# akosiorek/sqair

Measured on AMD Instinct MI355X. Metric: frames/sec (forward IWAE ELBO, 10-step 50x50 moving glyphs, K=5), higher is better.
Workload: dtype f32; 1 GPU; cfg2: T=10 HxW=50x50 B=32/GPU K=5 N=4 cells VanillaRNN/GRU/GRU forward (elbo_iwae), HIP-graph replay=True; global_batch=32, seq_len=10, parallelism=dp1, graph_nodes=879

## Files before the change

### sqair_amd/_capi.py

```python
from __future__ import annotations

import ctypes as C
import os

_HERE = os.path.dirname(os.path.abspath(__file__))
LIB_PATH = os.path.join(_HERE, "libsqair_hip.so")

OUTPUT_FIELDS = [
    "what", "what_loc", "what_scale", "where", "where_loc", "where_scale", "presence_prob", "presence",
    "presence_logit", "obj_id", "step_log_prob", "canvas", "glimpse", "disc_what_log_prob",
    "disc_where_log_prob", "disc_what_prior_log_prob", "disc_where_prior_log_prob", "disc_log_prob",
    "disc_prior_log_prob", "disc_prob", "prop_what_log_prob", "prop_where_log_prob",
    "prop_what_prior_log_prob", "prop_where_prior_log_prob", "prop_log_prob", "prop_prior_log_prob",
    "prop_prob", "discrete_log_prob", "num_prop_steps_per_sample", "num_disc_steps_per_sample",
    "num_steps_per_sample", "prop_pres", "disc_pres", "data_ll_per_sample", "kl_per_sample",
    "log_q_z_given_x_per_sample", "log_p_z_per_sample", "log_weights_per_timestep",
    "final_temporal_state", "final_prior_state", "final_last_used_id",
]
N_REFERENCE_OUTPUTS = 38


class SqairConfig(C.Structure):
    _fields_ = [
        ("img_h", C.c_int32), ("img_w", C.c_int32), ("glimpse_size", C.c_int32),
# ... 126 lines not shown
    "sqair_fill_noise": (C.c_int, [C.c_void_p, C.c_void_p, C.c_int, C.c_int, C.c_int, C.c_int, C.c_uint64, C.c_uint64, C.c_void_p]),
    "sqair_capture_begin": (C.c_int, [C.c_void_p, C.c_void_p]),
    "sqair_capture_end": (C.c_int, [C.c_void_p, C.c_void_p, C.c_int]),
    "sqair_capture_launch": (C.c_int, [C.c_void_p, C.c_int, C.c_void_p]),
    "sqair_add_l2_grad": (C.c_int, [C.c_void_p, C.c_void_p, C.c_void_p, C.c_int64, C.c_float, C.c_void_p]),
    "sqair_rmsprop_step": (C.c_int, [C.c_void_p, C.c_void_p, C.c_void_p, C.c_void_p, C.c_void_p, C.c_int64, C.c_float,
                                     C.c_float, C.c_float, C.c_float, C.c_float, C.c_void_p]),
    "sqair_linear_bwd_test": (C.c_int, [C.c_void_p] * 8 + [C.c_int] * 4 + [C.c_void_p, C.c_int64, C.c_void_p]),
    "sqair_debug_linear_time": (C.c_int, [C.c_void_p, C.c_void_p, C.c_void_p, C.c_void_p, C.c_void_p, C.c_int, C.c_int, C.c_int, C.c_int,
                                          C.c_void_p, C.c_int64, C.c_int, C.POINTER(C.c_float), C.c_void_p]),
    "sqair_debug_linear_graph_time": (C.c_int, [C.c_void_p, C.c_void_p, C.c_void_p, C.c_void_p, C.c_void_p, C.c_int, C.c_int, C.c_int, C.c_int,
                                              C.c_void_p, C.c_int64, C.c_int, C.c_int, C.c_int, C.POINTER(C.c_float), C.c_void_p]),
    "sqair_debug_dense_log": (C.c_int, [C.c_void_p, C.c_int]),
    "sqair_debug_dense_log_entry": (C.c_int, [C.c_void_p, C.c_int, C.POINTER(C.c_int)]),
    "sqair_debug_specialised_launches": (C.c_int64, []),
    "sqair_debug_layers": (C.c_int, [C.c_void_p]),
    "sqair_debug_padded_count": (C.c_int64, [C.c_void_p, C.POINTER(C.c_int)]),
    "sqair_debug_layer": (C.c_int, [C.c_void_p, C.c_int, C.POINTER(C.c_int), C.POINTER(C.c_int),
                                    C.POINTER(C.c_int), C.POINTER(C.c_int), C.POINTER(C.c_int)]),
    "sqair_debug_plan": (C.c_int, [C.c_void_p, C.c_int, C.POINTER(C.c_int), C.POINTER(C.c_int),
                                   C.POINTER(C.c_int)]),
}

EXPORTED_SYMBOLS = [n for n in _PROTOS if not n.startswith("sqair_debug")]

TIMELINE_LIB_PATH = os.path.join(_HERE, "libsqair_hip_timeline.so")
WIDE_LIB_PATH = os.path.join(_HERE, "libsqair_hip_wide.so")
PRODUCT_LIMITS = dict(n_what=50, n_steps_per_image=8, n_hidden=256)
WIDE_LIMITS = dict(n_what=128, n_steps_per_image=14, n_hidden=512)

# ... 74 lines not shown
```

### sqair_amd/csrc/sqair_api.hip

```cpp
#include <algorithm>
#include <mutex>
#include <set>
#include <utility>

#include "sqair_internal.h"
#include "sqair_chain.h"

void sq_set_error(SqairHandle* h, const std::string& msg) {
  if (h) h->err = msg;
}

struct PDim {
  std::vector<std::pair<int, int>> seg;
  PDim(int n) { seg.push_back({n, n}); }
  PDim(int t, int p) { seg.push_back({t, p}); }
  int t() const { int n = 0; for (auto& s : seg) n += s.first; return n; }
  int p() const { int n = 0; for (auto& s : seg) n += s.second; return n; }
  std::vector<int> map() const {
    std::vector<int> m;
    int base = 0;
    for (auto& s : seg) { for (int i = 0; i < s.first; ++i) m.push_back(base + i); base += s.second; }
    return m;
  }
};
// ... 173 lines not shown
  r[rec::PRES] = pres_row;
  return r;
}

struct SegSrc {
  std::string w;
  RowMap rows;
};
struct ColBlock {
  int ncols;
  int col0;
  std::vector<SegSrc> seg;
  std::string bias_a, bias_b;
};

static void build_layer(SqairHandle* h, LayerId id, const std::vector<int>& seg_width, const std::vector<ColBlock>& blocks) {
  PackedLayer& L = h->layers[id];
  L.seg_width = seg_width;
  L.kc = 0;
  for (int w : seg_width) L.kc += (w + 15) / 16;
  L.N = 0;
  for (const ColBlock& b : blocks) L.N += b.ncols;
  L.nt = (L.N + 15) / 16;
  L.w_off = h->packed_w;
  L.b_off = h->packed_b;
  const int64_t nel = (int64_t)L.nt * L.kc * 256;
  h->widx.resize(h->packed_w + nel, -1);
  h->bidx_a.resize(h->packed_b + L.nt * 16, -1);
  h->bidx_b.resize(h->packed_b + L.nt * 16, -1);
  int n0 = 0;
  for (const ColBlock& b : blocks) {
// ... 26 lines not shown
          for (int k = 0; k < seg_width[s]; ++k) {
            if (src.rows[k] < 0) continue;
            const int c = cbase + k / 16, kin = k % 16;
            const int lane = (kin / 4) * 16 + ln, comp = kin % 4;
            h->widx[L.w_off + (((int64_t)tile * L.kc + c) * 64 + lane) * 4 + comp] =
                (int)(woff + (int64_t)src.rows[k] * ldw + b.col0 + j);
          }
        }
        cbase += nch;
      }
    }
    n0 += b.ncols;
  }
  h->packed_w += nel;
  h->packed_b += L.nt * 16;
}

static ColBlock cb1(int ncols, int col0, const std::string& w, const RowMap& rows, const std::string& ba = "",
                    const std::string& bb = "") {
  ColBlock b;
  b.ncols = ncols;
  b.col0 = col0;
  b.seg.push_back({w, rows});
  b.bias_a = ba;
  b.bias_b = bb;
  return b;
}

static void build_plan(SqairHandle* h) {
  const SqairConfig& c = h->cfg;
// ... 49 lines not shown
    build_layer(h, L_PRIOR_GRU2, {nh}, {cb1(16, 0, "prop.prior_rnn.h2h.w", rm_none(nh))});
  } else {
    const RowMap zx = rm_zrec(nw, nw, 0, -1);
    std::vector<ColBlock> bl;
    const char* g[3] = {"z", "r", "h"};
    for (int i = 0; i < 3; ++i) {
      ColBlock b;
      b.ncols = nh;
      b.col0 = 0;
      b.seg.push_back({std::string("prop.prior_gru.w") + g[i], zx});
      if (i < 2) b.seg.push_back({std::string("prop.prior_gru.u") + g[i], rm_range(0, nh)});
      else b.seg.push_back({"", RowMap()});
      b.bias_a = std::string("prop.prior_gru.b") + g[i];
      bl.push_back(b);
    }
    build_layer(h, L_PRIOR_GRU1, {rec::ZW, nh}, bl);
    simple(L_PRIOR_GRU2, "prop.prior_gru.uh", nh, nh, 0, false);
  }
  simple(L_PRIOR_LIN, "prop.prior_linear", nh, 2 * (4 + nw) + 1);
  build_layer(h, L_TAU1, {nh},
              {cb1(128, 0, "prop.where_bias.l0.w", rm_range(0, nh), "prop.where_bias.l0.b"),
               cb1(128, 0, "enc.mask.l0.w", rm_range(0, nh), "enc.mask.l0.b")});
  simple(L_WB2, "prop.where_bias.l1", 128, 4);
  simple(L_MASK2, "enc.mask.l1", 128, G2);
  simple(L_GENC0, "enc.glimpse.l0", G2, nh);
  simple(L_GENC1, "enc.glimpse.l1", nh, nh);
  build_layer(h, L_WHAT_LOC, {nh}, {cb1(nw, 0, "enc.what_head.w", rm_range(0, nh), "enc.what_head.b")});
  simple(L_WHAT_HEAD, "enc.what_head", nh, 2 * nw);
  {
    std::vector<ColBlock> bl;
    for (int cc = 0; cc < nw; ++cc) {
// ... 19 lines not shown
    if (c.time_cell == CELL_VANILLA) {
      ColBlock u;
      u.ncols = nh; u.col0 = 0;
      u.seg = {{"", RowMap()}, {"", RowMap()}, {"prop.temporal_rnn.h2h.w", rm_range(0, nh)}};
      u.bias_a = "prop.temporal_rnn.i2h.b"; u.bias_b = "prop.temporal_rnn.h2h.b";
      bl.push_back(u);
    }
    for (const char* g : {"z", "r"}) {
      if (c.time_cell != CELL_GRU) break;
      ColBlock u;
      u.ncols = nh; u.col0 = 0;
      u.seg = {{"", RowMap()}, {"", RowMap()}, {std::string("prop.temporal_gru.u") + g, rm_range(0, nh)}};
      u.bias_a = std::string("prop.temporal_gru.b") + g;
      bl.push_back(u);
    }
    build_layer(h, L_PRE, {nw, rec::ZW, nh}, bl);
  }
  {
    build_layer(h, L_PROP_RNN, {rec::ZW, nh}, rnn_blocks("prop", {rm_zrec(nw, nw + nw, nw, nw + nw + 4), RowMap()}, 1, false, fin_p));
    if (RG) simple(L_PROP_RNN2, "prop.rnn_gru.uh", nh, nh, 0, false);
    else build_layer(h, L_PROP_RNN2, {nh}, {cb1(16, 0, "prop.what_head.w", rm_none(nh))});
  }
  build_layer(h, L_PROP_T1, {nh},
              {cb1(nh, 0, "prop.transform.l0.w", rm_range(0, nh)), cb1(nsp, 0, "prop.steps.l0.w", rm_range(0, nh))});
  simple(L_PROP_T2, "prop.transform.l1", nh, nh);
  simple(L_PROP_T3, "prop.transform.l2", nh, 8);
  if (c.time_cell == CELL_LSTM) {
    const std::string w = "prop.temporal_lstm.w";
    const int fin = nh + 4 + 2 * nw;
    ColBlock b;
    b.ncols = 4 * nh; b.col0 = 0;
// ... 340 lines not shown
  w.chain_ctl = (unsigned*)take(w.chain ? (int64_t)SQ_CHAIN_MAX_LAUNCHES * SQ_CHAIN_CTL_WORDS : 64);
  w.total = o;
  return w;
}
static Workspace carve(const SqairHandle* h, int T, int B, float* base) { return sq_carve(h, T, B, base, false); }

extern "C" int64_t sqair_workspace_bytes(const SqairHandle* h, int T, int B) {
  if (!h || T < 1 || B < 1) return -1;
  return sq_carve(h, T, B, nullptr, false).total * 4;
}
extern "C" int64_t sqair_train_workspace_bytes(const SqairHandle* h, int T, int B) {
  if (!h || T < 1 || B < 1) return -1;
  return sq_carve(h, T, B, nullptr, true).total * 4;
}

int sq_run(SqairHandle* h, Lin& l, LayerId id, int M, const float* packed, hipStream_t s) {
  const PackedLayer& L = h->layers[id];
  const PackedLayout pl = packed_layout(h);
  if (l.a.nseg != (int)L.seg_width.size()) {
    sq_set_error(h, "internal: segment count mismatch in layer " + std::to_string((int)id));
    return -3;
  }
  for (int i = 0; i < l.a.nseg; ++i)
    if (l.a.seg[i].width != L.seg_width[i]) {
      sq_set_error(h, "internal: segment width mismatch in layer " + std::to_string((int)id));
      return -3;
    }
  l.a.wp = packed + pl.w + L.w_off;
  l.a.wzero = packed + pl.w;
  l.a.bias = packed + pl.b + L.b_off;
  l.a.M = M;
  l.a.N = L.N;
  if (h->dense_log_on) { const int e[4] = {(int)id, M, L.kc * 16, L.N}; h->dense_log.insert(h->dense_log.end(), e, e + 4); }
  if (sq_chain_active(h)) return sq_chain_add_dense(h, l.a, L.kc, L.nt);
  const int rc = sq_launch_linear(l.a, L, s);
  if (rc != 0) sq_set_error(h, "internal: A-operand contract (16-byte aligned, ld % 4 == 0) violated in layer " + std::to_string((int)id));
  return rc;
}

static bool can_fuse_tail(const SqairHandle* h, LayerId id) {
  const PackedLayer& L = h->layers[id];
  const int nh = h->cfg.n_hidden;
  return h->cfg.rnn_cell == RNN_VANILLA && (nh == 128 || nh == 256) && L.seg_width.size() == 2 && L.seg_width[0] == rec::ZW &&
         L.seg_width[1] == nh && L.kc == 4 + nh / 16 && L.nt == nh / 16 && L.N == nh && h->opt_tail_fusion;
}
static int run_rnn_tail(SqairHandle* h, const TailArgs& ta, Dims d, LayerId id, const float* hid, int hid_ld, const float* add, int add_ld,
                        float* out, int out_ld, const float* packed, hipStream_t s) {
  const PackedLayer& L = h->layers[id];
  const PackedLayout pl = packed_layout(h);
  if (h->dense_log_on) { const int e[4] = {-1 - (int)id, d.R, L.kc * 16, L.N}; h->dense_log.insert(h->dense_log.end(), e, e + 4); }
// ... 351 lines not shown
    }
    if (w.chain) {
      const int rc = sq_chain_flush(h, w.chain_ctl + (size_t)(2 * t) * SQ_CHAIN_CTL_WORDS, 2 * t, s);
      if (rc != 0) return rc;
    }
    const bool do_generate = c.sample_from_prior && c.generate_after > 0 && (t_offset + t) > c.generate_after;
    GenArgs ga; memset(&ga, 0, sizeof(ga));
    if (c.sample_from_prior) {
      ga.rec_p = rec_p_t; ga.rec_d = rec_d_t; ga.rec_prev = rec_prev; ga.pstats = pstats_t; ga.ps_ld = PS_LD; ga.spre = spre_t;
      ga.gen_noise = h->gen_noise + (size_t)t * R * 2 * N * nzw; ga.gen = w.gen + (size_t)t * M * gen::W; ga.flat = flat;
      ga.do_generate = do_generate ? 1 : 0; ga.cfg = c;
      sq_launch_generate_prop(ga, po, d, s);
    }
    {
      Lin a; a.seg(rec_p_t, RW, rec::ZW).out(lea, nh).act(ACT_ELU); RUN(a, L_LAT0, M);
      Lin b; b.seg(lea, nh, nh).out(leb, nh).act(ACT_ELU); RUN(b, L_LAT1, M);
      sq_launch_latent_sum(leb, rec_p_t, cvec, d, s);
      Lin p; p.seg(cvec, nh, nh).add(w.pre_disc + (size_t)t * B * rw, rw, rw, K).out(w.pre_d, rw); RUN(p, L_PRED, R);
      if (c.rec_where_prior) {
        Lin q; q.seg(w.rn_init_state, 0, 4).seg(cvec, nh, nh).out(spre_t, 128); RUN(q, L_RNCOND, R);
      }
    }
    if (w.chain) sq_chain_begin(h, d, po, wsbase, ws_bytes);
    for (int j = 0; j < N; ++j) {
      {
        CropArgs ca; memset(&ca, 0, sizeof(ca));
        ca.mode = CROP_DISC;
        const int rc = slot_front(disc, j, ca, !fw);
        if (rc != 0) return rc;
      }
      if (fw) {
        const int rc = run_what(h, 0, w.slot(w.e2, nh, t, 1, j), w.sld(nh), R, j, nz, nullptr, 0, nullptr, rec_d_t, packed, s);
// ... 210 lines not shown
  if (h) sq_set_error(h, "sqair_timeline_begin: this library was built without -DSQAIR_TIMELINE (use libsqair_hip_timeline.so)");
  return -3;
}
extern "C" int sqair_timeline_count(const SqairHandle*) { return -3; }
extern "C" int sqair_timeline_end(SqairHandle*) { return -3; }
extern "C" int sqair_timeline_record(const SqairHandle*, int, const char**, int64_t*, int*, int*) { return -3; }
#endif

extern "C" int sqair_set_option(SqairHandle* h, const char* name, int value) {
  if (!h || !name) return -1;
  const std::string n(name);
  if (n == "tail_fusion") { h->opt_tail_fusion = value != 0; return 0; }
  if (n == "what_fusion") { h->opt_what_fusion = value != 0; return 0; }
  if (n == "specialised") { h->opt_specialised = value != 0; return 0; }
  if (n == "specialised_mask") { h->opt_specialised_mask = value; return 0; }
  if (n == "vi_target") {
    if (value != 0 && value != 1) { sq_set_error(h, "sqair_set_option: vi_target is 0 (vimco) or 1 (reinforce)"); return -2; }
    h->opt_vi_target = value;
    return 0;
  }
  if (n == "slot_chain") {
#ifdef SQAIR_WIDE
    if (value != 0) { sq_set_error(h, "sqair_set_option: slot_chain is not available in the wide build"); return -2; }
#endif
    h->opt_slot_chain = value != 0;
    h->opt_slot_chain_mode = value;
    return 0;
  }
  if (n == "slot_chain_arena_kb") {
    if (sq_chain_set_arena_kb(h, value) != 0) { sq_set_error(h, "sqair_set_option: slot_chain_arena_kb is 64 .. 1048576, set before the first pass"); return -2; }
    return 0;
  }
  sq_set_error(h, "sqair_set_option: unknown option '" + n + "' (known: tail_fusion, what_fusion, specialised, specialised_mask, slot_chain, slot_chain_arena_kb, vi_target)");
  return -2;
}

__global__ __launch_bounds__(256) void k_finite_check(const float* __restrict__ x, int64_t n, int* __restrict__ flag SQ_TLP) {
  SQ_TL_SCOPE;
  int bad = 0;
  int64_t first = n;
  for (int64_t i = (int64_t)blockIdx.x * 256 + threadIdx.x; i < n; i += (int64_t)gridDim.x * 256) {
    const float v = x[i];
    if (!(fabsf(v) <= 3.4028234664e38f)) { ++bad; if (i < first) first = i; }
  }
  if (bad) {
    atomicAdd(&flag[0], bad);
    atomicMin(&flag[1], (int)(first < 0x7fffffff ? first : 0x7fffffff));
  }
// ... 455 lines not shown
  hipStream_t s = (hipStream_t)stream;
  Dims d = make_dims(h->cfg, B);
  d.spec = h->opt_specialised && sq_spec_ok(d) ? (h->opt_specialised_mask & SPEC_ALL) : 0;
  CompactArgs ka; memset(&ka, 0, sizeof(ka));
  ka.rec_p = rec_p; ka.rec_d = rec_d; ka.rec_prev = rec_prev; ka.temporal_p = temporal_p; ka.prior_p = prior_p;
  ka.last_id_prev = last_id_prev; ka.last_id_next = last_id_next;
  ka.rec_next = rec_next; ka.temporal_next = temporal_next; ka.prior_next = prior_next;
  ka.flat = flat; ka.t = t; ka.out = *out; ka.src_out = src_out;
  sq_launch_compact(ka, h->po, d, s);
  SQ_CHECK_HIP(hipGetLastError());
  SQ_CHECK_HIP(hipStreamSynchronize(s));
  return 0;
}

extern "C" int64_t sqair_debug_specialised_launches(void) { return (int64_t)sq_spec_launches(); }
extern "C" int sqair_debug_layers(const SqairHandle* h) { return h ? (int)L_COUNT : -1; }
extern "C" int64_t sqair_debug_padded_count(const SqairHandle* h, int* u2i) {
  if (!h) return -1;
  if (u2i) memcpy(u2i, h->u2i.data(), h->u2i.size() * sizeof(int));
  return h->n_params;
}
extern "C" int sqair_debug_layer(const SqairHandle* h, int id, int* kc, int* nt, int* n, int* nseg, int* seg_widths) {
  if (!h || id < 0 || id >= L_COUNT) return -1;
  const PackedLayer& L = h->layers[id];
  *kc = L.kc; *nt = L.nt; *n = L.N; *nseg = (int)L.seg_width.size();
  for (size_t i = 0; i < L.seg_width.size() && i < 4; ++i) seg_widths[i] = L.seg_width[i];
  return 0;
}
extern "C" int sqair_debug_plan(const SqairHandle* h, int id, int* widx, int* bidx_a, int* bidx_b) {
  if (!h || id < 0 || id >= L_COUNT) return -1;
// ... 156 lines not shown
```

### sqair_amd/csrc/sqair_common.h

```cpp
#pragma once
#include <hip/hip_runtime.h>
#include <stdint.h>
#include <string>
#include <vector>

#include "../../include/sqair_hip.h"

#define SQ_CHECK_HIP(expr)                                                                   \
  do {                                                                                       \
    hipError_t _e = (expr);                                                                  \
    if (_e != hipSuccess) {                                                                  \
      sq_set_error(h, std::string(#expr) + ": " + hipGetErrorString(_e));                    \
      return -2;                                                                             \
    }                                                                                        \
  } while (0)

namespace rec {
#ifdef SQAIR_WIDE
constexpr int NWMAX = 128;
constexpr int WHERE = 0;
constexpr int WHAT = 4;
constexpr int PRES = 132;
constexpr int LOGIT = 133;
constexpr int ZW = 134;
// ... 58 lines not shown
  const float* e0; int e0_ld;
  const float* e1; int e1_ld;
  float* o1; int o1_ld;
  float* o2; int o2_ld;
  float* o3; int o3_ld;
  int nh;
};

struct PackedLayer {
  int64_t w_off;
  int64_t b_off;
  int kc;
  int nt;
  int N;
  std::vector<int> seg_width;
};

struct SqairHandle;
void sq_set_error(SqairHandle* h, const std::string& msg);
int sq_allow_big_lds(const void* kernel, int bytes);

__device__ __forceinline__ void philox4x32_10(unsigned c0, unsigned c1, unsigned c2, unsigned c3, unsigned k0, unsigned k1,
                                              unsigned out[4]) {
#pragma unroll
  for (int r = 0; r < 10; ++r) {
    const unsigned long long p0 = (unsigned long long)0xD2511F53u * c0, p1 = (unsigned long long)0xCD9E8D57u * c2;
    const unsigned n0 = (unsigned)(p1 >> 32) ^ c1 ^ k0, n1 = (unsigned)p1, n2 = (unsigned)(p0 >> 32) ^ c3 ^ k1, n3 = (unsigned)p0;
    c0 = n0; c1 = n1; c2 = n2; c3 = n3;
    k0 += 0x9E3779B9u; k1 += 0xBB67AE85u;
  }
  out[0] = c0; out[1] = c1; out[2] = c2; out[3] = c3;
}

int sq_launch_linear(const LinArgs& a, const PackedLayer& L, hipStream_t s);
int sq_launch_pack(const float* flat, float* packed_w, const int* idx, int64_t n, hipStream_t s);
int sq_launch_pack_bias(const float* flat, float* packed_b, const int* idxa, const int* idxb, int64_t n,
                        hipStream_t s);

#ifdef SQAIR_TIMELINE
struct SqTl { unsigned long long* slot; unsigned gx, gy, nw, pad; };
SqTl sq_tl_next(const char* kernel, dim3 grid, dim3 block);
#define SQ_TLP , const SqTl sq_tl
#define SQ_TL_SCOPE SqTlScope sq_tl_scope(sq_tl)
#define SQ_LAUNCH(kern, grid, block, lds, s, ...) \
  hipLaunchKernelGGL(kern, grid, block, lds, s, __VA_ARGS__, sq_tl_next(#kern, grid, block))
#ifdef __HIPCC__
struct SqTlScope {
  const SqTl tl;
  const unsigned long long t0;
// ... 151 lines not shown
```

### sqair_amd/csrc/sqair_glue.hip

```cpp
#include <atomic>

#include "sqair_glue.h"
#include "sqair_rowops.h"
#include "sqair_canvas.h"

__global__ void k_init_state(float* __restrict__ rec_m, float* __restrict__ temporal_m, float* __restrict__ prior_m,
                             float* __restrict__ last_id, float* __restrict__ disc_init_rec,
                             float* __restrict__ prop_rnn_init, float* __restrict__ disc_rnn_init,
                             float* __restrict__ rn_init_state, float* __restrict__ w3_prop,
                             float* __restrict__ w3_disc, int w3p_off, int w3d_off,
                             const float* __restrict__ flat, POff po, Dims d SQ_TLP) {
  SQ_TL_SCOPE;
  const int rs = blockIdx.x;
  const int tid = threadIdx.x;
  for (int i = tid; i < rec::W; i += blockDim.x) rec_m[(size_t)rs * rec::W + i] = (i == rec::ID) ? -1.0f : 0.0f;
  for (int i = tid; i < d.snh; i += blockDim.x) temporal_m[(size_t)rs * d.snh + i] = flat[po.temporal_init + i];
  for (int i = tid; i < d.psnh; i += blockDim.x) prior_m[(size_t)rs * d.psnh + i] = flat[po.prior_init + i];
  if (tid == 0 && (rs % d.N) == 0) last_id[rs / d.N] = -1.0f;
  if (rs == 0) {
    if (tid == 0) disc_init_rec[rec::PRES] = 1.0f;
    for (int i = tid; i < d.rsnh; i += blockDim.x) {
      prop_rnn_init[i] = flat[po.prop_rnn_init + i];
      disc_rnn_init[i] = flat[po.disc_rnn_init + i];
    }
// ... 835 lines not shown
  const dim3 g(nt, mt);
  if (d.nh == 256) SQ_RT(4, 1);
  else if (d.nh == 128) SQ_RT(2, 1);
  else return -1;
#undef SQ_RT
  return 0;
#endif
}

__global__ void k_latent_sum(const float* __restrict__ f, const float* __restrict__ rec_p, float* __restrict__ c, Dims d SQ_TLP) {
  SQ_TL_SCOPE;
  const int r = blockIdx.x;
  for (int n = threadIdx.x; n < d.nh; n += blockDim.x) {
    float acc = 0.0f;
    for (int k = 0; k < d.N; ++k)
      acc += f[((size_t)r * d.N + k) * d.nh + n] * rec_p[((size_t)r * d.N + k) * rec::W + rec::PRES];
    c[(size_t)r * d.nh + n] = acc;
  }
}
int sq_launch_latent_sum(const float* f, const float* rec_p, float* c, Dims d, hipStream_t s) {
  SQ_LAUNCH(k_latent_sum, dim3(d.R), dim3(256), 0, s, f, rec_p, c, d);
  return 0;
}

constexpr int SQ_LOGPROB_WAVES = 2;
__global__ __launch_bounds__(64 * SQ_LOGPROB_WAVES) void k_logprob(const LogprobArgs a, const POff po, const Dims d SQ_TLP) {
  SQ_TL_SCOPE;
  extern __shared__ __attribute__((aligned(16))) float smem[];
  const int r = blockIdx.x;
  const int fr = blockIdx.y;
  const int tid = threadIdx.x;
// ... 1203 lines not shown
```

### sqair_amd/csrc/sqair_internal.h

```cpp
#pragma once
#include <cstdio>
#include <cstring>
#include <map>

#include "sqair_glue.h"

struct ParamEntry {
  std::string name;
  int64_t off, numel;
  int rows, cols;
};

enum LayerId {
  L_IENC0, L_IENC1, L_PREDISC, L_PRIOR_GRU1, L_PRIOR_GRU2, L_PRIOR_LIN, L_TAU1, L_WB2, L_MASK2, L_GENC0, L_GENC1,
  L_WHAT_LOC, L_WHAT_HEAD, L_PRE, L_PROP_RNN, L_PROP_T1, L_PROP_T2, L_PROP_T3, L_PROP_GRU1, L_PROP_GRU2,
  L_PROP_HEADS, L_PROP_S1, L_LAT0, L_LAT1, L_PRED, L_RNCOND, L_DISC_RNN, L_DISC_T1, L_DISC_T2, L_DISC_T3,
  L_DISC_S1, L_DEC0, L_DEC1, L_DEC2, L_PROP_RNN2, L_DISC_RNN2,
  L_WHAT_HEAD_I, L_PROP_HEADS_I,
  L_COUNT
};

struct SqairHandle {
  SqairConfig cfg;
  SqairConfig ucfg;
// ... 18 lines not shown
  int64_t packed_w = 0, packed_b = 0;
  bool plan_uploaded_to = false;
  const void* plan_uploaded_ptr = nullptr;
  hipGraph_t graph = nullptr;
  hipGraphExec_t graph_exec = nullptr;
  int graph_nodes = 0;
  int debug_reps = 0;
  int debug_graph_nodes = 0;
  bool debug_graph_dependent = false;
  bool dense_log_on = false;
  std::vector<int> dense_log;
  float debug_us = 0.0f;
  bool opt_what_fusion = true;
  bool opt_specialised = true;
  int opt_specialised_mask = 3;
  bool opt_tail_fusion = true;
  bool opt_slot_chain = false;
  int opt_slot_chain_mode = 0;
  int opt_vi_target = 0;
  void* chain = nullptr;
  bool clear_each_pass = true;
  const float* gen_noise = nullptr;
  bool state_on = false;
  const void* state_in = nullptr;
  void* state_out = nullptr;
  const int32_t* state_src = nullptr;
  int state_B = 0;
  bool smc_on = false;
  SqairSmc smc = {};
  bool hist_on = false;
// ... 131 lines not shown
                                 int* t_row, float* fresh, int t0);
SQ_LOCAL int sq_history_refusal(SqairHandle* h, int T, int B, const SqairOutputs* outp);
SQ_LOCAL int sq_observed_refusal(SqairHandle* h, bool train, int T);
SQ_LOCAL HistPushArgs sq_history_push_args(const SqairHandle* h, const SqStateRes& st, const SqairOutputs& out, const int* t_row, int T, int B);
SQ_LOCAL SmcArgs sq_smc_args(const SqairSmc& m, const float* lw, const int32_t* t_row, int T, int B, int K);
SQ_LOCAL int sq_prior_step(SqairHandle* h, const float* packed, hipStream_t s, int M, const float* rec_prev, const float* prior_prev,
                           float* prior_p, float* pgz, float* pgrh, float* pgxh, float* pstats, float* o3, float* o1);

void sq_zero_fill(float* p, int64_t n, hipStream_t s);
void sq_copy(float* dst, const float* src, int64_t n, hipStream_t s);

inline const float* sq_flat(const SqairHandle* h, const float* user_flat, const void* packed) {
  return h->padded ? (const float*)packed + packed_layout(h).fi : user_flat;
}
void sq_flat_gather(const SqairHandle* h, const float* padded_grad, float* user_grad, const void* packed, hipStream_t s);
int sq_run(SqairHandle* h, Lin& l, LayerId id, int M, const float* packed, hipStream_t s);
#define RUN(l, id, M)                                   \
  do {                                                  \
    int _rc = sq_run(h, (l), (id), (M), packed, s);     \
    if (_rc != 0) return _rc;                           \
  } while (0)
```

### sqair_amd/csrc/sqair_linear.hip

```cpp
#include <type_traits>
#include "sqair_common.h"
#include "sqair_lin_device.h"
#include <stdio.h>
#include <stdlib.h>

typedef float f32x4 __attribute__((ext_vector_type(4)));

__global__ void k_pack(const float* __restrict__ flat, float* __restrict__ packed, const int* __restrict__ idx,
                       int64_t n SQ_TLP) {
  SQ_TL_SCOPE;
  constexpr int U = 8;
  int64_t i = (int64_t)blockIdx.x * blockDim.x + threadIdx.x;
  const int64_t stride = (int64_t)gridDim.x * blockDim.x;
  for (; i < n; i += stride * U) {
    int j[U];
    float v[U];
#pragma unroll
    for (int u = 0; u < U; ++u) j[u] = idx[min(i + u * stride, n - 1)];
#pragma unroll
    for (int u = 0; u < U; ++u) v[u] = flat[max(j[u], 0)];
#pragma unroll
    for (int u = 0; u < U; ++u)
      if (i + u * stride < n) packed[i + u * stride] = j[u] >= 0 ? v[u] : 0.0f;
  }
// ... 15 lines not shown
  if (blocks > 4096) blocks = 4096;
  SQ_LAUNCH(k_pack, dim3(blocks), dim3(256), 0, s, flat, packed_w, idx, n);
  return 0;
}
int sq_launch_pack_bias(const float* flat, float* packed_b, const int* idxa, const int* idxb, int64_t n,
                        hipStream_t s) {
  if (n <= 0) return 0;
  SQ_LAUNCH(k_pack_bias, dim3((unsigned)((n + 255) / 256)), dim3(256), 0, s, flat, packed_b, idxa, idxb, n);
  return 0;
}


#define SQ_KLINEAR_NAME k_linear
#include "sqair_linear_kernel.inc"
#undef SQ_KLINEAR_NAME

template <int NCH>
__global__ __launch_bounds__(256) void k_linear_rows(const LinArgs a, const int kc_total, const int n_tiles SQ_TLP) {
  SQ_TL_SCOPE;
  const int tid = threadIdx.x;
  const int wave = tid >> 6;
  const int lane = tid & 63;
  const int tile_n = blockIdx.x;
  const int tile_m = blockIdx.y * 4 + wave;
  (void)n_tiles;
  const int arow = min(tile_m * 16 + (lane & 15), a.M - 1);
  const int kq = lane >> 4;

  const int n = tile_n * 16 + (lane & 15);
  const int nc = min(n, a.N - 1);
// ... 669 lines not shown
  const dim3 g(L.nt, (a.M + 15) / 16);
#define SQ_LAUNCH_KL(G) SQ_LAUNCH((k_linear<NCH, NSEG, G>), g, dim3(256), 0, s, a.seg[0].p, a.wp, a.seg[0].ld, a.seg[0].width, a.seg[0].rmul, a.M, L.kc, L.nt, a.wzero, a)
  if (a.epi == EPI_ACT) SQ_LAUNCH_KL(false); else SQ_LAUNCH_KL(true);
#undef SQ_LAUNCH_KL
}
template <int NCH>
static void launch_nch(const LinArgs& a, const PackedLayer& L, hipStream_t s) {
  switch (a.nseg) {
    case 1: launch_seg<NCH, 1>(a, L, s); break;
    case 2: launch_seg<NCH, 2>(a, L, s); break;
    case 3: launch_seg<NCH, 3>(a, L, s); break;
    default: launch_seg<NCH, 4>(a, L, s); break;
  }
}

static unsigned rmul_of(int rdiv) { return rdiv <= 1 ? 0u : (unsigned)((1ull << 32) / (unsigned)rdiv) + 1u; }

int sq_launch_linear(const LinArgs& a_in, const PackedLayer& L, hipStream_t s) {
  LinArgs a = a_in;
  for (int i = 0; i < a.nseg; ++i) a.seg[i].rmul = rmul_of(a.seg[i].rdiv);
  a.add_rmul = rmul_of(a.add_rdiv);
  const int mt = (a.M + 15) / 16;
  const int grid = mt * L.nt;
  if (grid <= 0) return 0;
  for (int i = 0; i < a.nseg; ++i) {
    const LinSeg& sg = a.seg[i];
    if ((reinterpret_cast<uintptr_t>(sg.p) & 15) != 0 || (sg.ld & 3) != 0 || sg.width < 1 || sg.rdiv < 1) return -5;
  }
#ifndef SQAIR_MT_ROWS_DEFAULT
#define SQAIR_MT_ROWS_DEFAULT 6000
#endif
  static const int mt_rows = SQ_KNOB_INT("SQAIR_MT_ROWS", SQAIR_MT_ROWS_DEFAULT);
  const bool mid_wide = L.kc > 4 && a.M >= 1792 && L.nt >= 48;
// ... 27 lines not shown
    if (((a.M + 127) / 128) * ((L.nt + 3) / 4) >= lds_wgs) {
      SQ_LAUNCH((k_linear_lds<2>), dim3((L.nt + 3) / 4, (a.M + 127) / 128), dim3(256), 0, s, a, L.kc, L.nt);
      return 0;
    }
    const MtShape sh = pick_mt_shape(a.M, L.nt, L.kc);
    if (sh.nt >= 2) launch_mt<4, 1, 2>(a, L, mt, sh.coal != 0, s);
    else launch_mt<4, 1, 1>(a, L, mt, sh.coal != 0, s);
    return 0;
  }
  const int per_wave = (L.kc + 3) / 4;
  static const int t2_rows = SQ_KNOB_INT("SQAIR_T2_ROWS", 512), t2_kc = SQ_KNOB_INT("SQAIR_T2_KC", 40);
  if (a.M >= t2_rows && L.nt >= 4 && L.kc >= t2_kc) {
    launch_t2_any(a, L, s);
    return 0;
  }
  switch (per_wave) {
    case 1: launch_nch<1>(a, L, s); break;
    case 2: launch_nch<2>(a, L, s); break;
    case 3: launch_nch<3>(a, L, s); break;
    case 4: launch_nch<4>(a, L, s); break;
    case 5: launch_nch<5>(a, L, s); break;
    case 6: launch_nch<6>(a, L, s); break;
    case 7: launch_nch<7>(a, L, s); break;
    case 8: launch_nch<8>(a, L, s); break;
    case 9: launch_nch<9>(a, L, s); break;
    default: launch_nch<10>(a, L, s); break;
  }
  return 0;
}
```

### sqair_amd/csrc/sqair_linear_kernel.inc

```
template <int NCH, int NSEG = 4, bool GRU = true>
__global__ __launch_bounds__(256) void SQ_KLINEAR_NAME(const float* __restrict__ p0, const float* __restrict__ wp0, const int ld0,
                                                const int width0, const unsigned rmul0, const int M0, const int kc_total,
                                                const int n_tiles, const float* __restrict__ wzero0, const LinArgs a SQ_TLP) {
  SQ_TL_SCOPE;
  __shared__ float red[4 * 256];
  const int tid = threadIdx.x;
  const int wave = tid >> 6;
  const int lane = tid & 63;
#if defined(SQ_ROWTILE_XCD_AFFINITY)
  const int xcd = blockIdx.x & 7, qq = blockIdx.x >> 3;
  const int tile_n = qq % n_tiles;
  const int tile_m = xcd + 8 * (qq / n_tiles);
  if (tile_m * 16 >= a.M) return;
#else
  const int tile_n = blockIdx.x;
  const int tile_m = blockIdx.y;
  (void)n_tiles;
#endif
  const int arow = min(tile_m * 16 + (lane & 15), M0 - 1);
  const int kq = lane >> 4;

  const f32x4* __restrict__ wp = reinterpret_cast<const f32x4*>(wp0) + ((size_t)tile_n * kc_total) * 64 + lane;
  const int nmine = (kc_total - wave + 3) >> 2;
  const f32x4* __restrict__ wz = reinterpret_cast<const f32x4*>(wzero0) + lane;
  f32x4 av[NCH], bv[NCH];
#ifdef SQ_ABL_NO_B
#define SQ_KL_LOADB(p) f32x4{1.0f, 1.0f, 1.0f, 1.0f}
#else
#define SQ_KL_LOADB(p) *(p)
#endif
#define SQ_KL_ISSUE_B(BASE)                                                                                      \
  _Pragma("unroll") for (int j = 0; j < NCH; ++j) {                                                              \
    const bool valid = (BASE) + j < nmine;                                                                       \
    const int g = valid ? wave + 4 * ((BASE) + j) : wave;                                                        \
    bv[j] = SQ_KL_LOADB(valid ? wp + (size_t)g * 64 : wz);  \
  }
  if (NSEG > 1) {
    SQ_KL_ISSUE_B(0)
    __builtin_amdgcn_sched_barrier(0);
  }

  int cum1 = 0x7fffffff, cum2 = 0x7fffffff, cum3 = 0x7fffffff;
#define SQ_ROWOF(sg) ((sg).rmul ? (int)__umulhi((unsigned)arow, (sg).rmul) : arow)
  const float* rp0 = p0 + (size_t)(rmul0 ? (int)__umulhi((unsigned)arow, rmul0) : arow) * ld0;
  const float* rp1 = rp0; const float* rp2 = rp0; const float* rp3 = rp0;
  int lim0 = ((width0 + 3) & ~3) - 4, lim1 = 0, lim2 = 0, lim3 = 0;
  {
    int c = (width0 + 15) >> 4;
    if (NSEG > 1 && a.nseg > 1) { cum1 = c; c += (a.seg[1].width + 15) >> 4; rp1 = a.seg[1].p + (size_t)SQ_ROWOF(a.seg[1]) * a.seg[1].ld; lim1 = ((a.seg[1].width + 3) & ~3) - 4; }
    if (NSEG > 2 && a.nseg > 2) { cum2 = c; c += (a.seg[2].width + 15) >> 4; rp2 = a.seg[2].p + (size_t)SQ_ROWOF(a.seg[2]) * a.seg[2].ld; lim2 = ((a.seg[2].width + 3) & ~3) - 4; }
    if (NSEG > 3 && a.nseg > 3) { cum3 = c; rp3 = a.seg[3].p + (size_t)SQ_ROWOF(a.seg[3]) * a.seg[3].ld; lim3 = ((a.seg[3].width + 3) & ~3) - 4; }
  }

#undef SQ_ROWOF
  f32x4 acc0 = {0.0f, 0.0f, 0.0f, 0.0f}, acc1 = {0.0f, 0.0f, 0.0f, 0.0f};
#ifdef SQ_ABL_NO_A
#define SQ_KL_LOADA(p) f32x4{1.0f, 1.0f, 1.0f, 1.0f}
#else
#define SQ_KL_LOADA(p) *reinterpret_cast<const f32x4*>(p)
#endif
#define SQ_KL_ISSUE(BASE, FIRST)                                                                                 \
  _Pragma("unroll") for (int j = 0; j < NCH; ++j) {                                                              \
    const bool valid = (BASE) + j < nmine;                                                                       \
    const int g = valid ? wave + 4 * ((BASE) + j) : wave;  \
    const bool s1 = NSEG > 1 && g >= cum1, s2 = NSEG > 2 && g >= cum2, s3 = NSEG > 3 && g >= cum3;  \
    const float* rp = s3 ? rp3 : (s2 ? rp2 : (s1 ? rp1 : rp0));                                                  \
    const int cb = s3 ? cum3 : (s2 ? cum2 : (s1 ? cum1 : 0));                                                    \
    const int lim = s3 ? lim3 : (s2 ? lim2 : (s1 ? lim1 : lim0));                                                \
    av[j] = SQ_KL_LOADA(rp + min((g - cb) * 16 + kq * 4, lim));                                                  \
    if (!((FIRST) && NSEG > 1)) bv[j] = SQ_KL_LOADB(valid ? wp + (size_t)g * 64 : wz);                           \
  }
#ifndef SQ_ABL_NO_MFMA
#define SQ_KL_MFMA()                                                                                             \
  _Pragma("unroll") for (int j = 0; j < NCH; ++j) {                                                              \
    acc0 = __builtin_amdgcn_mfma_f32_16x16x4f32(av[j].x, bv[j].x, acc0, 0, 0, 0);                                \
    acc1 = __builtin_amdgcn_mfma_f32_16x16x4f32(av[j].y, bv[j].y, acc1, 0, 0, 0);                                \
    acc0 = __builtin_amdgcn_mfma_f32_16x16x4f32(av[j].z, bv[j].z, acc0, 0, 0, 0);                                \
    acc1 = __builtin_amdgcn_mfma_f32_16x16x4f32(av[j].w, bv[j].w, acc1, 0, 0, 0);                                \
  }
// ... 12 lines not shown
  const bool g2 = GRU && a.epi == EPI_GRU2;
  const int mcd = a.add_rmul ? (int)__umulhi((unsigned)mc, a.add_rmul) : mc;
  const float* pa = use_add ? a.add + (size_t)mcd * a.add_ld + nc : pb;
  const float* pe0 = g1 ? a.e0 + (size_t)mc * a.e0_ld + (nc - a.nh) : (g2 ? a.e0 + (size_t)mc * a.e0_ld + nc : pb);
  const float* pe1 = g2 ? a.e1 + (size_t)mc * a.e1_ld + nc : pb;
  const float* psc = a.scale_ptr != nullptr ? a.scale_ptr : pb;
#ifdef SQ_ABL_NO_EPI
  const float p_bias = 0.0f; float p_add = 0.0f; const float p_e0 = 0.0f, p_e1 = 0.0f; float p_scale = 1.0f;
  (void)pa; (void)pe0; (void)pe1; (void)psc;
#else
  const float p_bias = *pb;
  float p_add = *pa;
  const float p_e0 = *pe0, p_e1 = *pe1;
  float p_scale = *psc;
#endif
  p_add = use_add ? p_add : 0.0f;
  p_scale = a.scale_ptr != nullptr ? p_scale : 1.0f;
  const int e_split = a.act_split, e_acta = a.act_a, e_actb = a.act_b, e_ld = a.out_ld;
  float* const e_out = a.out;
  const float e_scale = a.scale;
  asm volatile("" ::"s"(e_split), "s"(e_acta), "s"(e_actb), "s"(e_ld), "s"(e_out), "s"(e_scale));

  __builtin_amdgcn_sched_barrier(0);
  SQ_KL_MFMA()
  if (NCH == 10) {
#pragma unroll 1
    for (int base = NCH; base < nmine; base += NCH) {
      SQ_KL_ISSUE(base, false)
      __builtin_amdgcn_sched_barrier(0);
      SQ_KL_MFMA()
    }
  }
#undef SQ_KL_ISSUE
#undef SQ_KL_ISSUE_B
#undef SQ_KL_MFMA
#undef SQ_KL_LOADA
#undef SQ_KL_LOADB

#if defined(SQ_PREFETCH_NEXT_W)
  if (a.e1 != nullptr) {
    const float* nw = a.e1 + ((size_t)tile_n * kc_total) * 256 + tid * 4;
#pragma unroll
    for (int q = 0; q < 4; ++q) {
      f32x4 junk;
      asm volatile("global_load_dwordx4 %0, %1, off" : "=v"(junk) : "v"(nw + (size_t)q * 1024 * (kc_total / 4)) : "memory");
    }
  }
#endif
  float* r = red + wave * 256;
  r[(4 * kq + 0) * 16 + (lane & 15)] = acc0.x + acc1.x;
  r[(4 * kq + 1) * 16 + (lane & 15)] = acc0.y + acc1.y;
  r[(4 * kq + 2) * 16 + (lane & 15)] = acc0.z + acc1.z;
  r[(4 * kq + 3) * 16 + (lane & 15)] = acc0.w + acc1.w;
  __syncthreads();
  if (live) {
    float v = red[tid] + red[256 + tid] + red[512 + tid] + red[768 + tid] + p_bias + p_add;
    if (!GRU || a.epi == EPI_ACT) {
      v = sq_act(v, n < e_split ? e_acta : e_actb);
      e_out[(size_t)m * e_ld + n] = v * e_scale * p_scale;
    } else if (a.epi == EPI_GRU1) {
      const int nh = a.nh;
      if (n < nh) a.out[(size_t)m * a.out_ld + n] = sq_sigmoid(v);
      else if (n < 2 * nh) {
        const float rg = sq_sigmoid(v);
        a.o1[(size_t)m * a.o1_ld + (n - nh)] = rg * p_e0;
        if (a.o3 != nullptr) a.o3[(size_t)m * a.o3_ld + (n - nh)] = rg;
      }
      else a.o2[(size_t)m * a.o2_ld + (n - 2 * nh)] = v;
    } else {
// ... 8 lines not shown
```

Before: 101,700 frames/s.

## Skip all-zero K chunks per tile class and fuse latent sum into linear

Adds a ranged linear kernel that, for the prior GRU1 and PRE layers, restricts each output tile to the K-chunk range with nonzero packed weights, described by up to three tile classes. It also adds a fused latsum variant of the linear kernel that applies the ELU epilogue and computes the presence-weighted slot sum directly in the epilogue. That fusion removes the separate latent-sum launch and, in inference, the write of the intermediate features. Both are enabled by default through new frame_trim options. The costs are extra kernel instantiations, an extra syncthreads and shared-memory use in the fused epilogue, and reliance on the packed-weight sparsity structure.

```diff
diff --git a/sqair_amd/_capi.py b/sqair_amd/_capi.py
--- a/sqair_amd/_capi.py
+++ b/sqair_amd/_capi.py
@@ -164,6 +164,8 @@
     "sqair_debug_dense_log": (C.c_int, [C.c_void_p, C.c_int]),
     "sqair_debug_dense_log_entry": (C.c_int, [C.c_void_p, C.c_int, C.POINTER(C.c_int)]),
     "sqair_debug_specialised_launches": (C.c_int64, []),
+    "sqair_debug_ranged_launches": (C.c_int64, []),
+    "sqair_debug_layer_ranges": (C.c_int, [C.c_void_p, C.c_int, C.POINTER(C.c_int)]),
     "sqair_debug_layers": (C.c_int, [C.c_void_p]),
     "sqair_debug_padded_count": (C.c_int64, [C.c_void_p, C.POINTER(C.c_int)]),
     "sqair_debug_layer": (C.c_int, [C.c_void_p, C.c_int, C.POINTER(C.c_int), C.POINTER(C.c_int),
diff --git a/sqair_amd/csrc/sqair_api.hip b/sqair_amd/csrc/sqair_api.hip
--- a/sqair_amd/csrc/sqair_api.hip
+++ b/sqair_amd/csrc/sqair_api.hip
@@ -211,7 +211,7 @@
   std::string bias_a, bias_b;
 };
 
-static void build_layer(SqairHandle* h, LayerId id, const std::vector<int>& seg_width, const std::vector<ColBlock>& blocks) {
+static void build_layer(SqairHandle* h, LayerId id, const std::vector<int>& seg_width, const std::vector<ColBlock>& blocks, bool ranges = false) {
   PackedLayer& L = h->layers[id];
   L.seg_width = seg_width;
   L.kc = 0;
@@ -268,6 +268,34 @@
   }
   h->packed_w += nel;
   h->packed_b += L.nt * 16;
+  L.rg_n = 0;
+  L.rg[0] = L.rg[1] = L.rg[2] = 0;
+  if (ranges && L.kc <= 255 && L.nt < 0x7fff) {
+    int n_cls = 0, cls_b[3], cls_e[3], cls_t0[3];
+    bool ok = true;
+    for (int tile = 0; tile < L.nt && ok; ++tile) {
+      int kb = L.kc, ke = 0;
+      for (int c = 0; c < L.kc; ++c) {
+        const int64_t o = L.w_off + ((int64_t)tile * L.kc + c) * 256;
+        bool any = false;
+        for (int e = 0; e < 256 && !any; ++e) any = h->widx[o + e] >= 0;
+        if (any) { kb = std::min(kb, c); ke = c + 1; }
+      }
+      if (ke == 0) kb = 0;
+      kb &= ~3;
+      if (n_cls > 0 && cls_b[n_cls - 1] == kb && cls_e[n_cls - 1] == ke) continue;
+      if (n_cls == 3) { ok = false; break; }
+      cls_b[n_cls] = kb; cls_e[n_cls] = ke; cls_t0[n_cls] = tile; ++n_cls;
+    }
+    if (ok && n_cls > 1) {
+      L.rg_n = n_cls;
+      for (int i = 0; i < 3; ++i) {
+        const int j = std::min(i, n_cls - 1);
+        const int next = i + 1 < n_cls ? cls_t0[i + 1] : 0x7fff;
+        L.rg[i] = cls_b[j] | (cls_e[j] << 8) | (next << 16);
+      }
+    }
+  }
 }
 
 static ColBlock cb1(int ncols, int col0, const std::string& w, const RowMap& rows, const std::string& ba = "",
@@ -347,7 +375,7 @@
       b.bias_a = std::string("prop.prior_gru.b") + g[i];
       bl.push_back(b);
     }
-    build_layer(h, L_PRIOR_GRU1, {rec::ZW, nh}, bl);
+    build_layer(h, L_PRIOR_GRU1, {rec::ZW, nh}, bl, true);
     simple(L_PRIOR_GRU2, "prop.prior_gru.uh", nh, nh, 0, false);
   }
   simple(L_PRIOR_LIN, "prop.prior_linear", nh, 2 * (4 + nw) + 1);
@@ -397,7 +425,7 @@
       u.bias_a = std::string("prop.temporal_gru.b") + g;
       bl.push_back(u);
     }
-    build_layer(h, L_PRE, {nw, rec::ZW, nh}, bl);
+    build_layer(h, L_PRE, {nw, rec::ZW, nh}, bl, true);
   }
   {
     build_layer(h, L_PROP_RNN, {rec::ZW, nh}, rnn_blocks("prop", {rm_zrec(nw, nw + nw, nw, nw + nw + 4), RowMap()}, 1, false, fin_p));
@@ -768,7 +796,7 @@
   return sq_carve(h, T, B, nullptr, true).total * 4;
 }
 
-int sq_run(SqairHandle* h, Lin& l, LayerId id, int M, const float* packed, hipStream_t s) {
+int sq_run(SqairHandle* h, Lin& l, LayerId id, int M, const float* packed, hipStream_t s, const LatSum* ls, bool* ls_done) {
   const PackedLayer& L = h->layers[id];
   const PackedLayout pl = packed_layout(h);
   if (l.a.nseg != (int)L.seg_width.size()) {
@@ -787,7 +815,7 @@
   l.a.N = L.N;
   if (h->dense_log_on) { const int e[4] = {(int)id, M, L.kc * 16, L.N}; h->dense_log.insert(h->dense_log.end(), e, e + 4); }
   if (sq_chain_active(h)) return sq_chain_add_dense(h, l.a, L.kc, L.nt);
-  const int rc = sq_launch_linear(l.a, L, s);
+  const int rc = sq_launch_linear(l.a, L, s, h->opt_frame_trim && (h->opt_frame_trim_mask & 1) != 0, ls, ls_done);
   if (rc != 0) sq_set_error(h, "internal: A-operand contract (16-byte aligned, ld % 4 == 0) violated in layer " + std::to_string((int)id));
   return rc;
 }
@@ -1169,8 +1197,12 @@
     }
     {
       Lin a; a.seg(rec_p_t, RW, rec::ZW).out(lea, nh).act(ACT_ELU); RUN(a, L_LAT0, M);
-      Lin b; b.seg(lea, nh, nh).out(leb, nh).act(ACT_ELU); RUN(b, L_LAT1, M);
-      sq_launch_latent_sum(leb, rec_p_t, cvec, d, s);
+      LatSum ls; memset(&ls, 0, sizeof(ls));
+      ls.pres = rec_p_t + rec::PRES; ls.pres_ld = RW; ls.c = cvec; ls.c_ld = nh; ls.n_slots = N; ls.rows = R; ls.write_f = train ? 1 : 0;
+      bool summed = false;
+      Lin b; b.seg(lea, nh, nh).out(leb, nh).act(ACT_ELU);
+      { const int rc = sq_run(h, b, L_LAT1, M, packed, s, h->opt_frame_trim && (h->opt_frame_trim_mask & 4) ? &ls : nullptr, &summed); if (rc != 0) return rc; }
+      if (!summed) sq_launch_latent_sum(leb, rec_p_t, cvec, d, s);
       Lin p; p.seg(cvec, nh, nh).add(w.pre_disc + (size_t)t * B * rw, rw, rw, K).out(w.pre_d, rw); RUN(p, L_PRED, R);
       if (c.rec_where_prior) {
         Lin q; q.seg(w.rn_init_state, 0, 4).seg(cvec, nh, nh).out(spre_t, 128); RUN(q, L_RNCOND, R);
@@ -1411,6 +1443,8 @@
   if (n == "what_fusion") { h->opt_what_fusion = value != 0; return 0; }
   if (n == "specialised") { h->opt_specialised = value != 0; return 0; }
   if (n == "specialised_mask") { h->opt_specialised_mask = value; return 0; }
+  if (n == "frame_trim") { h->opt_frame_trim = value != 0; return 0; }
+  if (n == "frame_trim_mask") { h->opt_frame_trim_mask = value; return 0; }
   if (n == "vi_target") {
     if (value != 0 && value != 1) { sq_set_error(h, "sqair_set_option: vi_target is 0 (vimco) or 1 (reinforce)"); return -2; }
     h->opt_vi_target = value;
@@ -1428,7 +1462,7 @@
     if (sq_chain_set_arena_kb(h, value) != 0) { sq_set_error(h, "sqair_set_option: slot_chain_arena_kb is 64 .. 1048576, set before the first pass"); return -2; }
     return 0;
   }
-  sq_set_error(h, "sqair_set_option: unknown option '" + n + "' (known: tail_fusion, what_fusion, specialised, specialised_mask, slot_chain, slot_chain_arena_kb, vi_target)");
+  sq_set_error(h, "sqair_set_option: unknown option '" + n + "' (known: tail_fusion, what_fusion, specialised, specialised_mask, frame_trim, frame_trim_mask, slot_chain, slot_chain_arena_kb, vi_target)");
   return -2;
 }
 
@@ -1914,6 +1948,13 @@
 }
 
 extern "C" int64_t sqair_debug_specialised_launches(void) { return (int64_t)sq_spec_launches(); }
+extern "C" int64_t sqair_debug_ranged_launches(void) { return (int64_t)sq_ranged_launches(); }
+extern "C" int sqair_debug_layer_ranges(const SqairHandle* h, int id, int* rg) {
+  if (!h || !rg || id < 0 || id >= L_COUNT) return -1;
+  const PackedLayer& L = h->layers[id];
+  for (int i = 0; i < 3; ++i) rg[i] = L.rg[i];
+  return L.rg_n;
+}
 extern "C" int sqair_debug_layers(const SqairHandle* h) { return h ? (int)L_COUNT : -1; }
 extern "C" int64_t sqair_debug_padded_count(const SqairHandle* h, int* u2i) {
   if (!h) return -1;
diff --git a/sqair_amd/csrc/sqair_common.h b/sqair_amd/csrc/sqair_common.h
--- a/sqair_amd/csrc/sqair_common.h
+++ b/sqair_amd/csrc/sqair_common.h
@@ -96,6 +96,15 @@
   int nt;
   int N;
   std::vector<int> seg_width;
+  int rg_n = 0;
+  int rg[3] = {0, 0, 0};
+};
+
+struct LatSum {
+  const float* pres; int pres_ld;
+  float* c; int c_ld;
+  int n_slots, per_tile, rows;
+  int write_f;
 };
 
 struct SqairHandle;
@@ -114,7 +123,8 @@
   out[0] = c0; out[1] = c1; out[2] = c2; out[3] = c3;
 }
 
-int sq_launch_linear(const LinArgs& a, const PackedLayer& L, hipStream_t s);
+int sq_launch_linear(const LinArgs& a, const PackedLayer& L, hipStream_t s, bool ranged = false, const LatSum* ls = nullptr, bool* ls_done = nullptr);
+long long sq_ranged_launches();
 int sq_launch_pack(const float* flat, float* packed_w, const int* idx, int64_t n, hipStream_t s);
 int sq_launch_pack_bias(const float* flat, float* packed_b, const int* idxa, const int* idxb, int64_t n,
                         hipStream_t s);
diff --git a/sqair_amd/csrc/sqair_glue.hip b/sqair_amd/csrc/sqair_glue.hip
--- a/sqair_amd/csrc/sqair_glue.hip
+++ b/sqair_amd/csrc/sqair_glue.hip
@@ -873,7 +873,7 @@
   for (int n = threadIdx.x; n < d.nh; n += blockDim.x) {
     float acc = 0.0f;
     for (int k = 0; k < d.N; ++k)
-      acc += f[((size_t)r * d.N + k) * d.nh + n] * rec_p[((size_t)r * d.N + k) * rec::W + rec::PRES];
+      acc = fmaf(f[((size_t)r * d.N + k) * d.nh + n], rec_p[((size_t)r * d.N + k) * rec::W + rec::PRES], acc);
     c[(size_t)r * d.nh + n] = acc;
   }
 }
diff --git a/sqair_amd/csrc/sqair_internal.h b/sqair_amd/csrc/sqair_internal.h
--- a/sqair_amd/csrc/sqair_internal.h
+++ b/sqair_amd/csrc/sqair_internal.h
@@ -56,6 +56,8 @@
   bool opt_what_fusion = true;
   bool opt_specialised = true;
   int opt_specialised_mask = 3;
+  bool opt_frame_trim = true;
+  int opt_frame_trim_mask = 5;
   bool opt_tail_fusion = true;
   bool opt_slot_chain = false;
   int opt_slot_chain_mode = 0;
@@ -217,7 +219,7 @@
   return h->padded ? (const float*)packed + packed_layout(h).fi : user_flat;
 }
 void sq_flat_gather(const SqairHandle* h, const float* padded_grad, float* user_grad, const void* packed, hipStream_t s);
-int sq_run(SqairHandle* h, Lin& l, LayerId id, int M, const float* packed, hipStream_t s);
+int sq_run(SqairHandle* h, Lin& l, LayerId id, int M, const float* packed, hipStream_t s, const LatSum* ls = nullptr, bool* ls_done = nullptr);
 #define RUN(l, id, M)                                   \
   do {                                                  \
     int _rc = sq_run(h, (l), (id), (M), packed, s);     \
diff --git a/sqair_amd/csrc/sqair_linear.hip b/sqair_amd/csrc/sqair_linear.hip
--- a/sqair_amd/csrc/sqair_linear.hip
+++ b/sqair_amd/csrc/sqair_linear.hip
@@ -1,3 +1,4 @@
+#include <atomic>
 #include <type_traits>
 #include "sqair_common.h"
 #include "sqair_lin_device.h"
@@ -53,6 +54,18 @@
 #define SQ_KLINEAR_NAME k_linear
 #include "sqair_linear_kernel.inc"
 #undef SQ_KLINEAR_NAME
+#define SQ_KLINEAR_NAME k_linear_ranged
+#define SQ_KL_RANGED
+#include "sqair_linear_kernel.inc"
+#undef SQ_KL_RANGED
+#undef SQ_KLINEAR_NAME
+#ifndef SQAIR_WIDE
+#define SQ_KLINEAR_NAME k_linear_latsum
+#define SQ_KL_LATSUM
+#include "sqair_linear_kernel.inc"
+#undef SQ_KL_LATSUM
+#undef SQ_KLINEAR_NAME
+#endif
 
 template <int NCH>
 __global__ __launch_bounds__(256) void k_linear_rows(const LinArgs a, const int kc_total, const int n_tiles SQ_TLP) {
@@ -752,9 +765,42 @@
   }
 }
 
+template <int NCH>
+static bool launch_ranged_nch(const LinArgs& a, const PackedLayer& L, hipStream_t s) {
+  const dim3 g(L.nt, (a.M + 15) / 16);
+#define SQ_LAUNCH_KLR(NSEG, G) SQ_LAUNCH((k_linear_ranged<NCH, NSEG, G>), g, dim3(256), 0, s, a.seg[0].p, a.wp, a.seg[0].ld, a.seg[0].width, a.seg[0].rmul, a.M, L.kc, L.nt, L.rg[0], L.rg[1], L.rg[2], a.wzero, a)
+  if (a.nseg == 3 && a.epi == EPI_ACT) { SQ_LAUNCH_KLR(3, false); return true; }
+  if (a.nseg == 2 && a.epi == EPI_GRU1) { SQ_LAUNCH_KLR(2, true); return true; }
+#undef SQ_LAUNCH_KLR
+  return false;
+}
+#ifndef SQAIR_WIDE
+template <int NCH>
+static void launch_latsum(const LinArgs& a, const PackedLayer& L, const LatSum& ls, hipStream_t s) {
+  SQ_LAUNCH((k_linear_latsum<NCH, 1, false>), dim3(L.nt, (a.M + 15) / 16), dim3(256), 0, s, a.seg[0].p, a.wp, a.seg[0].ld, a.seg[0].width,
+            a.seg[0].rmul, a.M, L.kc, L.nt, a.wzero, a, ls);
+}
+#endif
+static std::atomic<long long> g_ranged_launches{0};
+long long sq_ranged_launches() { return g_ranged_launches.load(); }
+static bool launch_ranged(const LinArgs& a, const PackedLayer& L, int per_wave, hipStream_t s) {
+  bool done = false;
+  switch (per_wave) {
+    case 3: done = launch_ranged_nch<3>(a, L, s); break;
+    case 4: done = launch_ranged_nch<4>(a, L, s); break;
+    case 5: done = launch_ranged_nch<5>(a, L, s); break;
+    case 6: done = launch_ranged_nch<6>(a, L, s); break;
+    case 7: done = launch_ranged_nch<7>(a, L, s); break;
+    case 8: done = launch_ranged_nch<8>(a, L, s); break;
+    default: break;
+  }
+  if (done) ++g_ranged_launches;
+  return done;
+}
+
 static unsigned rmul_of(int rdiv) { return rdiv <= 1 ? 0u : (unsigned)((1ull << 32) / (unsigned)rdiv) + 1u; }
 
-int sq_launch_linear(const LinArgs& a_in, const PackedLayer& L, hipStream_t s) {
+int sq_launch_linear(const LinArgs& a_in, const PackedLayer& L, hipStream_t s, bool ranged, const LatSum* ls, bool* ls_done) {
   LinArgs a = a_in;
   for (int i = 0; i < a.nseg; ++i) a.seg[i].rmul = rmul_of(a.seg[i].rdiv);
   a.add_rmul = rmul_of(a.add_rdiv);
@@ -812,6 +858,17 @@
     launch_t2_any(a, L, s);
     return 0;
   }
+  if (ranged && L.rg_n > 1 && launch_ranged(a, L, per_wave, s)) return 0;
+#ifndef SQAIR_WIDE
+  if (ls != nullptr && a.nseg == 1 && a.epi == EPI_ACT && (per_wave == 2 || per_wave == 4) && ls->n_slots >= 1 && 16 % ls->n_slots == 0 &&
+      a.M == ls->rows * ls->n_slots) {
+    LatSum l = *ls;
+    l.per_tile = 16 / l.n_slots;
+    if (per_wave == 2) launch_latsum<2>(a, L, l, s); else launch_latsum<4>(a, L, l, s);
+    *ls_done = true;
+    return 0;
+  }
+#endif
   switch (per_wave) {
     case 1: launch_nch<1>(a, L, s); break;
     case 2: launch_nch<2>(a, L, s); break;
diff --git a/sqair_amd/csrc/sqair_linear_kernel.inc b/sqair_amd/csrc/sqair_linear_kernel.inc
--- a/sqair_amd/csrc/sqair_linear_kernel.inc
+++ b/sqair_amd/csrc/sqair_linear_kernel.inc
@@ -1,7 +1,19 @@
+#ifdef SQ_KL_LATSUM
+#define SQ_KL_LATSUM_PARAMS , const LatSum ls
+#else
+#define SQ_KL_LATSUM_PARAMS
+#endif
+#ifdef SQ_KL_RANGED
+#define SQ_KL_RANGE_PARAMS const int rg0, const int rg1, const int rg2,
+#define SQ_KL_G(i) (k_begin + wave + 4 * (i))
+#else
+#define SQ_KL_RANGE_PARAMS
+#define SQ_KL_G(i) (wave + 4 * (i))
+#endif
 template <int NCH, int NSEG = 4, bool GRU = true>
 __global__ __launch_bounds__(256) void SQ_KLINEAR_NAME(const float* __restrict__ p0, const float* __restrict__ wp0, const int ld0,
                                                 const int width0, const unsigned rmul0, const int M0, const int kc_total,
-                                                const int n_tiles, const float* __restrict__ wzero0, const LinArgs a SQ_TLP) {
+                                                const int n_tiles, SQ_KL_RANGE_PARAMS const float* __restrict__ wzero0, const LinArgs a SQ_KL_LATSUM_PARAMS SQ_TLP) {
   SQ_TL_SCOPE;
   __shared__ float red[4 * 256];
   const int tid = threadIdx.x;
@@ -21,7 +33,13 @@
   const int kq = lane >> 4;
 
   const f32x4* __restrict__ wp = reinterpret_cast<const f32x4*>(wp0) + ((size_t)tile_n * kc_total) * 64 + lane;
+#ifdef SQ_KL_RANGED
+  const int rgw = tile_n < (rg0 >> 16) ? rg0 : (tile_n < (rg1 >> 16) ? rg1 : rg2);
+  const int k_begin = rgw & 255;
+  const int nmine = (((rgw >> 8) & 255) - k_begin - wave + 3) >> 2;
+#else
   const int nmine = (kc_total - wave + 3) >> 2;
+#endif
   const f32x4* __restrict__ wz = reinterpret_cast<const f32x4*>(wzero0) + lane;
   f32x4 av[NCH], bv[NCH];
 #ifdef SQ_ABL_NO_B
@@ -32,7 +50,7 @@
 #define SQ_KL_ISSUE_B(BASE)                                                                                      \
   _Pragma("unroll") for (int j = 0; j < NCH; ++j) {                                                              \
     const bool valid = (BASE) + j < nmine;                                                                       \
-    const int g = valid ? wave + 4 * ((BASE) + j) : wave;                                                        \
+    const int g = valid ? SQ_KL_G((BASE) + j) : wave;                                                        \
     bv[j] = SQ_KL_LOADB(valid ? wp + (size_t)g * 64 : wz);  \
   }
   if (NSEG > 1) {
@@ -62,7 +80,7 @@
 #define SQ_KL_ISSUE(BASE, FIRST)                                                                                 \
   _Pragma("unroll") for (int j = 0; j < NCH; ++j) {                                                              \
     const bool valid = (BASE) + j < nmine;                                                                       \
-    const int g = valid ? wave + 4 * ((BASE) + j) : wave;  \
+    const int g = valid ? SQ_KL_G((BASE) + j) : wave;  \
     const bool s1 = NSEG > 1 && g >= cum1, s2 = NSEG > 2 && g >= cum2, s3 = NSEG > 3 && g >= cum3;  \
     const float* rp = s3 ? rp3 : (s2 ? rp2 : (s1 ? rp1 : rp0));                                                  \
     const int cb = s3 ? cum3 : (s2 ? cum2 : (s1 ? cum1 : 0));                                                    \
@@ -105,6 +123,9 @@
   const float p_e0 = *pe0, p_e1 = *pe1;
   float p_scale = *psc;
 #endif
+#ifdef SQ_KL_LATSUM
+  const float ls_p = ls.pres[(size_t)mc * ls.pres_ld];
+#endif
   p_add = use_add ? p_add : 0.0f;
   p_scale = a.scale_ptr != nullptr ? p_scale : 1.0f;
   const int e_split = a.act_split, e_acta = a.act_a, e_actb = a.act_b, e_ld = a.out_ld;
@@ -127,6 +148,9 @@
 #undef SQ_KL_MFMA
 #undef SQ_KL_LOADA
 #undef SQ_KL_LOADB
+#undef SQ_KL_G
+#undef SQ_KL_RANGE_PARAMS
+#undef SQ_KL_LATSUM_PARAMS
 
 #if defined(SQ_PREFETCH_NEXT_W)
   if (a.e1 != nullptr) {
@@ -144,6 +168,29 @@
   r[(4 * kq + 2) * 16 + (lane & 15)] = acc0.z + acc1.z;
   r[(4 * kq + 3) * 16 + (lane & 15)] = acc0.w + acc1.w;
   __syncthreads();
+#ifdef SQ_KL_LATSUM
+  {
+    __shared__ float ls_f[256];
+    __shared__ float ls_ps[16];
+    float f = 0.0f;
+    if (live) {
+      const float v = red[tid] + red[256 + tid] + red[512 + tid] + red[768 + tid] + p_bias + p_add;
+      f = sq_act(v, n < e_split ? e_acta : e_actb) * e_scale * p_scale;
+      if (ls.write_f) e_out[(size_t)m * e_ld + n] = f;
+    }
+    ls_f[tid] = f;
+    if ((tid & 15) == 0) ls_ps[tid >> 4] = ls_p;
+    __syncthreads();
+    const int pr = tid >> 4;
+    const int r = tile_m * ls.per_tile + pr;
+    if (pr < ls.per_tile && r < ls.rows && n < a.N) {
+      float acc = 0.0f;
+      for (int k = 0; k < ls.n_slots; ++k) acc = fmaf(ls_f[(pr * ls.n_slots + k) * 16 + (tid & 15)], ls_ps[pr * ls.n_slots + k], acc);
+      ls.c[(size_t)r * ls.c_ld + n] = acc;
+    }
+    return;
+  }
+#endif
   if (live) {
     float v = red[tid] + red[256 + tid] + red[512 + tid] + red[768 + tid] + p_bias + p_add;
     if (!GRU || a.epi == EPI_ACT) {
```

Result: no change. 102,600 frames/s (median of 6 runs) (+0.9%).
